# maxjiang216/corintho-ai

Hardware: AMD Instinct MI355X
Metric: self-play games/sec at 400 sims/move (higher is better)
Workload: dtype f32(f16x3)

## Files before the change

### corintho_ai_amd/csrc/engine.hip

```cpp
#include <math.h>
#include <stdio.h>
#include <stdlib.h>
#include <string.h>

#include <algorithm>
#include <memory>
#include <string>
#include <vector>

#include "analysis_host.h"
#include "game_logs.h"
#include "game_store.h"
#include "game_view.h"
#include "net_host.h"
#include "nn_group.h"
#include "pools.h"
#include "samples_host.h"

#ifdef CO_EMU
thread_local int co_emu_block_idx = 0;
#ifdef CO_SB_STATS
unsigned long long co_sb_stats[32];
unsigned long long co_sb_ply[8][8];
extern "C" unsigned long long *co_emu_sb_stats(void) { return co_sb_stats; }
extern "C" unsigned long long *co_emu_sb_ply(void) { return &co_sb_ply[0][0]; }
#endif
#endif

thread_local std::string g_last_error;
extern "C" const char *ca_last_error(void) { return g_last_error.c_str(); }
void co_set_last_error(const std::string &m) { g_last_error = m; }

struct ca_trainer {
  ca_config cfg;
  int G = 0, spe = 0;
  Stream stream;
  EngineParams P;
  GameStore store;
  GameView view;
  GameLogs logs;
  SampleExits samples;
  HostForward host_forward;
  AnalysisPositions positions;
  TourneyTables tour;
  int64_t iterations = 0;
  int32_t trainer_iteration = 0;
  bool scan_valid = false;
  int scan_valid_for = 0;
  int32_t last_total = 0;
  bool finished = false;
  bool any_error = false;
  bool net_used = false;
  std::unique_ptr<CoNet> nets[2];
  CallbackState callback{false, false, " in this generation; it cannot go on -- start a new one with ca_trainer_reset"};
  RunStats stats;
  FusedRun fused;
  bool host_cache = false;
  int host_cache_log2 = -1;
  int32_t host_rows = 0;
  HostNet host_net;
  HostPins pins;

  int dev() const { return cfg.device; }
  bool self_play_training() const { return !cfg.testing && !cfg.analyse && !tour.active(); }
  bool use_cache() const {
    if (cfg.eval_cache < 0 || tour.active() || cfg.analyse) return false;
    if (cfg.eval_cache > 0) return true;
    return nets[0] && nets[0]->flop_per_row() >= 1e6;
  }
  void invalidate() { scan_valid = view.valid = false; }
  size_t request_rows() const { return store.request_rows(spe); }
  const std::vector<GameCtl> &games() { return view.fetch(store, G, stream); }

  void init(const ca_config &c, TourneyTables tables = TourneyTables()) {
    cfg = c;
    tour = std::move(tables);
    if (cfg.analyse) {
      cfg.testing = 1;
      cfg.no_stagger = 1;
      cfg.game_base = cfg.total_games = 0;
    }
    if (cfg.max_searches <= 0) cfg.max_searches = 1600;
    if (cfg.searches_per_eval <= 0) cfg.searches_per_eval = 16;
    if (cfg.c_puct <= 0.0f) cfg.c_puct = 1.0f;
    G = cfg.num_games;
    spe = cfg.searches_per_eval;
    rt_set_device(cfg.device);
    stream.create();
    store.create(cfg, G, spe, self_play_training(), cfg.eval_cache >= 0 && !tour.active() && !cfg.analyse, stream);
    if (tour.active()) tour.create(store.R, stream);
    if (!cfg.analyse) reset_games(cfg.seed);
    rebind();
    fused.work_counter = store.work_counter.p;
    fused.nn_eval = store.nn_eval.p;
    fused.nn_probs = store.nn_probs.p;
    fused.stats = &stats;
    fused.stream = stream;
  }

  void rebind() {
    memset(&P, 0, sizeof P);
    store.bind(P, cfg, G, spe);
    logs.bind(P);
    tour.bind(P);
  }

  void reset_games(int32_t seed) {
    cfg.seed = seed;
    if (positions.given()) positions.write_terminal_rows(store.req.p, (size_t)spe * CO_STATE_STRIDE, stream);
    store.seed(cfg, G, tour.active() ? tour.match_seeds.data() : positions.given() ? positions.seed.data() : nullptr,
               [&](GameCtl &gc, int g) {
                 if (positions.given()) positions.place(gc, g);
               },
               stream);
    iterations = 0;
    trainer_iteration = 0;
    invalidate();
    last_total = 0;
    host_rows = 0;
    finished = false;
    const int64_t cache_clears = stats.cache_clears;
    stats = RunStats();
    stats.cache_clears = cache_clears;
    fused.cache_clean = false;
    callback.failed = false;
    for (auto &n : nets)
      if (n) n->clear_failure();
    logs.clear(stream);
  }

  void set_logging(const char *folder, int n) {
    if (tour.active() || cfg.analyse) throw CaError(CA_ERR_STATE, "per-game logs belong to Trainer games (self-play or arena)");
    if (iterations != 0 || trainer_iteration != 0) throw CaError(CA_ERR_STATE, "ca_trainer_set_logging: the games have started");
    if (n < 0) throw CaError(CA_ERR_ARG, "ca_trainer_set_logging: num_logged < 0");
    n -= cfg.game_base;
    if (n < 0) n = 0;
    if (n > G) n = G;
    if (n > store.R)
      throw CaError(CA_ERR_ARG, "ca_trainer_set_logging: " + std::to_string(n) + " logged games on " + std::to_string(store.R) +
                                        " resident slots -- a logged game must start in its own slot; raise ca_config.resident");
    std::vector<int> first(n);
    for (int g = 0; g < n; ++g) first[g] = g;
    set_log_records(first, GameLogs::game_paths(folder, cfg.game_base, n), false);
  }
  void set_log_records(const std::vector<int> &which, const std::vector<std::string> &paths, bool with_index) {
    logs.set_records(which, paths, with_index, G, stream);
    rebind();
  }
  void write_logs_once() {
    if (logs.pending()) logs.write(games(), stream);
  }

  EngineParams params(int to_play) const {
    EngineParams e = P;
    e.to_play = to_play;
    e.iteration = trainer_iteration;
    return e;
  }

  void scan(const EngineParams &e) { RT_LAUNCH(co_k_scan, 1, CO_WAVE, stream, e); }
  void compact(const EngineParams &e) { RT_LAUNCH(co_k_compact, store.R, CO_WAVE, stream, e); }
  void read_ctl(int to_play) {
    last_total = store.h_ctl[CO_CTL_ROWS];
    finished = store.h_ctl[CO_CTL_ALL_DONE] != 0;
    any_error = store.h_ctl[CO_CTL_ANY_ERROR] != 0;
    scan_valid_for = to_play;
    scan_valid = true;
  }
  void pack(int to_play) {
    if (scan_valid && scan_valid_for == to_play) return;
    const EngineParams e = params(to_play);
    scan(e);
    compact(e);
    rt_d2h(store.h_ctl, store.ctl.p, CO_CTL_WORDS * 4, stream);
    rt_sync(stream);
    read_ctl(to_play);
    if (finished && !any_error) write_logs_once();
  }
  bool poll_all_done(int to_play) {
    scan(params(to_play));
    int32_t d = 0;
    rt_d2h(&d, store.all_done.p, 4, stream);
    rt_sync(stream);
    return d != 0;
  }

  bool upload_answers(const float *evals, const float *probs, int32_t rows) {
    if (rows <= 0 || !evals || !probs) return false;
    rt_h2d(store.nn_eval.p, evals, (size_t)rows * 4, stream);
    rt_h2d(store.nn_probs.p, probs, (size_t)rows * CO_NUM_MOVES * 4, stream);
    return true;
  }

  void check_errors() {
    check_net_range();
    if (scan_valid && !any_error) return;
    throw_game_errors(games());
  }

  void step(const EngineParams &e) {
    launch_mcts_step(e, store.R, stream);
    ++stats.mcts_launches;
    invalidate();
    pack(e.to_play);
    check_errors();
  }
  void queue_iteration(const EngineParams &e, CoNet *net) {
    scan(e);
    if (net) {
      compact(e);
      net->forward(store.nn_in.p, store.R * spe, store.req_offset.p + store.R, store.nn_eval.p, store.nn_probs.p, stream);
      ++stats.nn_launches;
    }
    launch_mcts_step(e, store.R, stream);
    ++stats.mcts_launches;
    ++iterations;
  }
  void queue_grouped_iteration(CoNetGroup *group, GroupPlanner &planner, const int32_t *slot_model, int32_t *row_model) {
    const EngineParams e = params(CO_TO_PLAY_EVERY_MODEL);
    scan(e);
    compact(e);
    RT_LAUNCH(co_k_group_rows, store.R, CO_WAVE, stream, e, slot_model, row_model);
    planner.run(row_model, store.req_offset.p + store.R, stream);
    group->forward(store.nn_in.p, store.R * spe, planner.plan(), store.nn_eval.p, store.nn_probs.p, stream);
    ++stats.nn_launches;
    launch_mcts_step(e, store.R, stream);
    ++stats.mcts_launches;
    ++iterations;
  }
  void queued_iterations_done() {
    invalidate();
    check_errors();
  }
  void drain() {
    rt_sync(stream);
    invalidate();
  }

  void need_positions() const {
    if (cfg.analyse && !positions.given()) throw CaError(CA_ERR_STATE, "analysis trainer: ca_trainer_set_positions first");
  }
  bool do_iteration(const float *evals, const float *probs, int to_play) {
    need_positions();
    callback.need_none_failed("ca_trainer_do_iteration");
    if (host_cache) return host_cache_iteration(evals, probs, to_play);
    if (iterations > 0) {
      pack(to_play);
      if (last_total > 0 && !upload_answers(evals, probs, last_total))
        throw CaError(CA_ERR_ARG, "doIteration: null evaluations/probabilities");
    } else {
      rt_memset(store.req_offset.p, 0, ((size_t)store.R + 1) * 4, stream);
    }
    const EngineParams e = params(to_play);
    if (to_play == -1) ++trainer_iteration;
    ++iterations;
    step(e);
    return finished;
  }

  int32_t num_requests(int to_play) {
    if (host_cache) return host_cache_all_games(to_play), host_rows;
    pack(to_play);
    return last_total;
  }

  void write_requests(float *out, int to_play) {
    const int32_t n = num_requests(to_play);
    if (n == 0) return;
    rt_d2h(out, store.nn_in70.p, (size_t)n * CO_GAME_STATE_SIZE * 4, stream);
    rt_sync(stream);
  }

  void set_host_cache(int32_t log2_entries) {
    if ((log2_entries >= 1 && log2_entries <= 5) || log2_entries > 30)
      throw CaError(CA_ERR_ARG, "ca_trainer_set_host_cache: log2_entries must be negative (off), 0 (automatic) or 6..30, not " +
                                        std::to_string(log2_entries));
    const bool on = log2_entries >= 0;
    if (on && !self_play_training())
      throw CaError(CA_ERR_STATE, "ca_trainer_set_host_cache: the evaluation cache serves self-play training only, not a testing, "
                                  "analysis or tournament trainer");
    if (!on && !host_cache) return;
    if (iterations != 0)
      throw CaError(CA_ERR_STATE, "ca_trainer_set_host_cache: in the middle of a generation; switch before the first "
                                  "ca_trainer_do_iteration or after ca_trainer_reset");
    fused.release();
    host_cache = on;
    host_cache_log2 = log2_entries;
    fused.host_stepped = on;
    host_rows = 0;
    if (!on) return;
    if (!store.pend_key.p) {
      store.alloc_pend_keys(spe, stream);
      rebind();
      rt_sync(stream);
    }
    fused.spe = spe;
    fused.create(1, store.R, log2_entries);
    fused.cache_clean = false;
    host_net.rows_cap = request_rows();
    host_net.rows70 = store.nn_in70.p;
    host_net.ev_in = store.nn_eval.p;
    host_net.pr_in = store.nn_probs.p;
    host_net.d_ctl = store.ctl.p;
    host_net.h_ctl = &store.h_ctl[0];
    host_net.out_idx = nullptr;
  }
  void host_cache_all_games(int to_play) const {
    if (to_play != -1) throw CaError(CA_ERR_ARG, "host-driven protocol with the evaluation cache: to_play must be -1 (training)");
  }
  bool host_cache_iteration(const float *evals, const float *probs, int to_play) {
    host_cache_all_games(to_play);
    rt_stream_t st = fused.pools[0].st;
    if (host_rows > 0) {
      if (!evals || !probs) throw CaError(CA_ERR_ARG, "doIteration: null evaluations/probabilities");
      host_net.receive(evals, probs, host_rows, st);
      host_rows = 0;
    }
    EngineParams e = params(-1);
    e.step_budget = 0;
    e.step_budget_k16 = 0;
    host_net.scan_params = e;
    const int64_t n = fused.run(e, &host_net, 1, host_cache_log2, iterations > 0, 1);
    trainer_iteration += (int32_t)n;
    iterations += n;
    invalidate();
    stats.estimate_device_times(true);
    if (!fused.failure.empty()) throw CaError(CA_ERR_ENGINE, fused.failure);
    read_ctl(-1);
    const Pool::Seen &seen = fused.pools[0].seen[0];
    host_rows = (int32_t)std::min<size_t>(seen.evaluated, request_rows());
    stats.nn_rows += (int64_t)co_pack_rows(seen.pack);
    stats.nn_rows_evaluated += host_rows;
    check_errors();
    if (finished) write_logs_once();
    return finished;
  }

  int32_t need_samples(const char *what, int32_t cap_rows = INT32_MAX) {
    if (cfg.testing) throw CaError(CA_ERR_STATE, std::string(what) + " in testing mode");
    return samples.index(games(), cap_rows, stream);
  }
  void write_samples(float *gs, float *ev, float *pr) {
    const size_t n = (size_t)need_samples("writeSamples");
    if (n > 0) samples.write(P, G, n, gs, ev, pr, stream);
  }
  int32_t pack_samples_device(float *d_state_policy, float *d_outcome, int32_t cap_rows) {
    const int32_t n = need_samples("pack_samples", cap_rows);
    if (n > cap_rows) throw CaError(CA_ERR_ARG, "pack_samples: destination too small");
    if (n > 0) samples.pack(P, G, d_state_policy, d_outcome, stream);
    rt_sync(stream);
    return n;
  }
  void export_samples(float *state_policy, float *outcome) {
    const size_t n = (size_t)need_samples("export_samples");
    if (n > 0) samples.export_host(P, G, n, state_policy, outcome, stream);
  }

  void set_positions(const int32_t *boards, const int32_t *to_play, const int32_t *pieces, const int32_t *seeds) {
    if (!cfg.analyse) throw CaError(CA_ERR_STATE, "set_positions: not an analysis trainer (ca_config.analyse)");
    if (iterations > 0) throw CaError(CA_ERR_STATE, "set_positions after the first iteration");
    positions.set(boards, to_play, pieces, seeds, G, stream);
    reset_games(cfg.seed);
  }
  void analysis(int32_t *out) {
    if (!cfg.analyse) throw CaError(CA_ERR_STATE, "not an analysis trainer");
    AnalysisPositions::read(store.req.p, (size_t)spe * CO_STATE_STRIDE, games(), out, stream);
  }
  void finish_analysis() {
    if (!cfg.analyse) throw CaError(CA_ERR_STATE, "ca_trainer_finish: not an analysis trainer");
    if (iterations == 0) do_iteration(nullptr, nullptr, -1);
    EngineParams e = params(-1);
    e.force_choose = 1;
    step(e);
  }

  std::unique_ptr<CoNet> make_net(const NetSpec &spec, CallbackState *guard, const std::string &asker, const char *hint = "") {
    return spec.make(request_rows(), stream, guard, asker, hint);
  }
  void set_net(int slot, const NetSpec &spec, const char *who) {
    if (slot < 0 || slot > 1) throw CaError(CA_ERR_ARG, "net slot must be 0 or 1");
    install_net(slot, make_net(spec, &callback, ", this trainer", " (ca_trainer_request_rows)"), who);
  }

  void install_net(int slot, std::unique_ptr<CoNet> fresh, const char *who) {
    if (slot == 0 && !fused.pools.empty() && !host_cache) {
      std::unique_ptr<CoNet> old = std::move(nets[0]);
      nets[0] = std::move(fresh);
      const bool toggles = (fused.table.entries != 0) != use_cache();
      if (toggles && iterations > 0 && !finished) {
        nets[0] = std::move(old);
        throw CaError(CA_ERR_STATE, std::string(who) + ": this network turns the evaluation cache " +
                                            std::string(fused.table.entries ? "off" : "on") +
                                            " in the middle of a generation; finish or reset the generation first");
      }
      if (toggles) fused.release();
    } else {
      nets[slot] = std::move(fresh);
    }
    if (slot == 0) fused.cache_clean = false;
  }

  void check_callback() {
    for (int slot = 0; slot < 2; ++slot)
      if (nets[slot] && nets[slot]->callback_failed()) invalidate(), callback.check(nets[slot].get(), "slot " + std::to_string(slot));
  }

  void check_net_range() {
    if (!net_used) return;
    for (int slot = 0; slot < 2; ++slot) ::check_net_range(nets[slot].get(), stream, "network slot " + std::to_string(slot));
    net_used = false;
  }

  void net_forward_host(int slot, const float *states, int32_t n, float *evals, float *probs) {
    if (slot < 0 || slot > 1 || !nets[slot]) throw CaError(CA_ERR_STATE, "net slot not set");
    callback.need_none_failed("ca_trainer_net_forward");
    CoNet *net = nets[slot].get();
// ... 302 lines not shown
```

### corintho_ai_amd/csrc/game_store.h

```cpp
#pragma once
#include <string.h>

#include <algorithm>
#include <random>
#include <vector>

#include "host.h"
#include "kernels.h"
#include "pools.h"

struct GameStore {
  int R = 0;
  bool recycle = false;
  uint32_t cap_units = 0;
  DevBuf<GameCtl> games;
  DevBuf<TreeCtl> trees;
  DevBuf<uint4> arena, pend_key;
  DevBuf<int32_t> pend_src;
  DevBuf<uint32_t> pend_leaf, pend_path, pend_n, noise_raw, rng;
  DevBuf<int32_t> pend_depth, req_offset, trace, all_done;
  DevBuf<float> req, nn_in, nn_in70, nn_eval, nn_probs, samples;
  DevBuf<int32_t> row_idx;
  DevBuf<unsigned long long> row_counter, pack_counter, work_counter, prof, next_game;
  DevBuf<GameCtl> results;
  DevBuf<uint32_t> seeds_dev;
  DevBuf<int32_t> arena_state;
  DevBuf<int32_t> ctl;
  Pinned<int32_t> h_ctl;

  size_t request_rows(int spe) const { return (size_t)R * spe; }

  void alloc_pend_keys(int spe, rt_stream_t s) {
    pend_key.alloc(request_rows(spe), s);
    pend_src.alloc(request_rows(spe), s);
  }

  void create(const ca_config &cfg, int G, int spe, bool can_recycle, bool cache_words, rt_stream_t s) {
    uint32_t cap = cfg.arena_units;
    if (cap == 0) {
      uint64_t nodes = (uint64_t)cfg.max_searches * 14 + 64;
      cap = (uint32_t)std::min<uint64_t>(nodes * 40, 0x7FFFFFF0ull);
    }
    cap_units = cap;
    R = G;
    const size_t per_slot = (size_t)2 * ((size_t)cap + CO_ARENA_PAD) * sizeof(uint4) +
                            (size_t)spe * (CO_PATH_MAX * 4 + CO_NUM_MOVES * 4 + 2 * CO_STATE_STRIDE * 4 + CO_GAME_STATE_SIZE * 4 +
                                           CO_NUM_MOVES * 4 + 64) + CO_MT_N * 4 + 512;
    if (can_recycle && cfg.resident > 0 && cfg.resident < G) R = cfg.resident;
    if (can_recycle && cfg.resident == 0) {
      const size_t budget = rt_mem_free() / 8 * 5;
      const size_t per_game = (size_t)CO_MAX_PLIES * CO_SAMPLE_FLOATS * 4 + sizeof(GameCtl) + 8;
      if ((size_t)G * (per_slot + per_game) > budget) {
        size_t fit = budget > (size_t)G * per_game ? (budget - (size_t)G * per_game) / per_slot : 0;
        if (fit < 1) throw CaError(CA_ERR_DEVICE, "not enough device memory for a single resident game");
        R = (int)std::min<size_t>(fit, (size_t)G);
        if (R >= 512) R &= ~255;
      }
    }
    recycle = R < G;
    const size_t T = (size_t)2 * R, rows = request_rows(spe);
    games.alloc(R, s);
    trees.alloc(T, s);
    arena.alloc(T * ((size_t)cap + CO_ARENA_PAD), s);
    pend_leaf.alloc(rows, s);
    pend_depth.alloc(rows, s);
    pend_n.alloc(rows * 4, s);
    if (cache_words) alloc_pend_keys(spe, s);
    noise_raw.alloc(rows * CO_NUM_MOVES, s);
    pend_path.alloc(rows * CO_PATH_MAX, s);
    rng.alloc((size_t)R * CO_MT_N, s);
    req.alloc(rows * CO_STATE_STRIDE, s);
    req_offset.alloc((size_t)R + 1, s);
    nn_in.alloc(rows * CO_STATE_STRIDE, s);
    row_idx.alloc(rows, s);
    nn_in70.alloc(rows * CO_GAME_STATE_SIZE, s);
    ctl.alloc(CO_CTL_WORDS, s);
    h_ctl.alloc(CO_CTL_WORDS);
    nn_eval.alloc(rows, s);
    nn_probs.alloc(rows * CO_NUM_MOVES, s);
    if (!cfg.testing) samples.alloc((size_t)G * CO_MAX_PLIES * CO_SAMPLE_FLOATS, s);
    if (cfg.trace) trace.alloc((size_t)G * CO_TRACE_CAP, s);
    if (recycle) {
      results.alloc(G, s);
      seeds_dev.alloc(G, s);
    }
    next_game.alloc(1, s);
    all_done.alloc(1, s);
    row_counter.alloc(1, s);
    pack_counter.alloc((size_t)CO_PACK_STRIDE * CO_MAX_POOLS, s);
    work_counter.alloc((size_t)CO_WC_WORDS * CO_MAX_POOLS, s);
    arena_state.alloc(CO_AS_WORDS, s);
#ifdef CO_PROF
    prof.alloc((size_t)R * CO_NPROF + 24 + CO_NPROF, s);
#endif
  }

  template <class F>
  void seed(const ca_config &cfg, int G, const uint32_t *given, F &&place, rt_stream_t s) {
    size_t T = (size_t)2 * R;
    int total = cfg.total_games > 0 ? cfg.total_games : G;
    std::mt19937 gen((uint32_t)cfg.seed);
    std::vector<uint32_t> seeds(total);
    for (int i = 0; i < total; ++i) seeds[i] = (uint32_t)gen();
    std::vector<uint32_t> st((size_t)R * CO_MT_N);
    std::vector<GameCtl> hg(R);
    std::vector<TreeCtl> ht(T);
    for (int g = 0; g < R; ++g) {
      uint32_t *x = &st[(size_t)g * CO_MT_N];
      x[0] = given ? given[g] : seeds[cfg.game_base + g];
      for (int i = 1; i < CO_MT_N; ++i) x[i] = 1812433253u * (x[i - 1] ^ (x[i - 1] >> 30)) + (uint32_t)i;
      memset(&hg[g], 0, sizeof(GameCtl));
      hg[g].gid = g;
      hg[g].parity = (cfg.game_base + g) % 2;
      hg[g].rng_idx = CO_MT_N;
      hg[g].pos_meta = CO_META_START;
      place(hg[g], g);
    }
    for (size_t t = 0; t < T; ++t) {
      ht[t].root = CO_NONE;
      ht[t].searches_done = 0;
      ht[t].units_used = 0;
      ht[t].peak_units = 0;
    }
    rt_h2d(rng.p, st.data(), st.size() * 4, s);
    rt_h2d(games.p, hg.data(), hg.size() * sizeof(GameCtl), s);
    rt_h2d(trees.p, ht.data(), ht.size() * sizeof(TreeCtl), s);
    if (recycle) {
      rt_h2d(seeds_dev.p, seeds.data() + cfg.game_base, (size_t)G * 4, s);
      rt_memset(results.p, 0, (size_t)G * sizeof(GameCtl), s);
    }
    const unsigned long long first_unstarted = (unsigned long long)R;
    rt_h2d(next_game.p, &first_unstarted, 8, s);
    rt_memset(row_counter.p, 0, 8, s);
    rt_memset(pack_counter.p, 0, (size_t)8 * CO_PACK_STRIDE * CO_MAX_POOLS, s);
    rt_memset(work_counter.p, 0, (size_t)8 * CO_WC_WORDS * CO_MAX_POOLS, s);
    rt_memset(arena_state.p, 0, CO_AS_WORDS * 4, s);
    rt_sync(s);
  }

  void bind(EngineParams &P, const ca_config &cfg, int G, int spe) const {
    P.num_games = R;
    P.total_local = G;
    P.results = recycle ? results.p : nullptr;
    P.next_game = next_game.p;
    P.seeds = recycle ? seeds_dev.p : nullptr;
    P.max_searches = cfg.max_searches;
    P.searches_per_eval = spe;
    P.c_puct = cfg.c_puct;
    P.epsilon = cfg.epsilon;
    P.testing = cfg.testing;
    size_t div = (size_t)(cfg.total_games > 0 ? cfg.total_games : G) / (size_t)cfg.max_searches;
    if (div < 1) div = 1;
    P.stagger_div = (cfg.no_stagger || recycle) ? 0 : (int32_t)div;
    P.iteration = 0;
    P.to_play = -1;
    P.game_base = cfg.game_base;
    P.cap_units = cap_units;
    P.trace_on = cfg.trace;
    P.analyse = cfg.analyse;
    P.arena_state = nullptr;
    P.scan_phase = 0;
    P.games = games.p;
    P.trees = trees.p;
    P.arena = arena.p;
    P.pend_leaf = pend_leaf.p;
    P.pend_depth = pend_depth.p;
    P.pend_n = pend_n.p;
    P.pend_key = pend_key.p;
    P.pend_src = pend_src.p;
    P.noise_raw = noise_raw.p;
    P.pend_path = pend_path.p;
    P.rng = rng.p;
    P.req = req.p;
    P.req_offset = req_offset.p;
    P.nn_eval = nn_eval.p;
    P.nn_probs = nn_probs.p;
    P.nn_in = nn_in.p;
    P.row_idx = row_idx.p;
    P.nn_in70 = nn_in70.p;
    P.ctl = ctl.p;
    P.samples = samples.p;
    P.trace = trace.p;
    P.all_done = all_done.p;
    P.row_counter = nullptr;
    P.fused_pack = 0;
    P.defer_handover = 0;
    P.step_budget = cfg.step_budget > 0 ? cfg.step_budget : 0;
    P.step_budget_k16 = cfg.step_budget == 0 ? CO_STEP_BUDGET_K16 : cfg.step_budget < -1 ? -cfg.step_budget : 0;
    P.work_counter = nullptr;
    P.pool_lo = 0;
    P.pool_n = R;
    P.pool_row_base = 0;
    P.pack_counter = pack_counter.p;
    P.prof = prof.p;
  }

  int64_t peak_arena_units(rt_stream_t s) const {
    std::vector<TreeCtl> ht((size_t)2 * R);
    rt_d2h(ht.data(), trees.p, ht.size() * sizeof(TreeCtl), s);
    rt_sync(s);
    int64_t peak = 0;
    for (auto &x : ht) peak = std::max<int64_t>(peak, x.peak_units);
    return peak;
  }

  void read_prof(unsigned long long out[2 * CO_NPROF + 24], rt_stream_t s) const {
    if (!prof.p) throw CaError(CA_ERR_STATE, "not a -DCO_PROF build");
    for (int i = 0; i < 2 * CO_NPROF + 24; ++i) out[i] = 0;
    std::vector<unsigned long long> h((size_t)R * CO_NPROF);
    rt_d2h(h.data(), prof.p, h.size() * 8, s);
    rt_sync(s);
    for (int g = 0; g < R; ++g)
      for (int i = 0; i < CO_NPROF; ++i) out[i] += h[(size_t)g * CO_NPROF + i];
    rt_d2h(out + CO_NPROF, prof.p + (size_t)R * CO_NPROF, (size_t)(24 + CO_NPROF) * 8, s);
    rt_sync(s);
  }
};

struct TourneyTables {
  std::vector<PlayerCfg> host_pcfg;
  std::vector<uint32_t> match_seeds;
  bool exact_offsets = false;
  DevBuf<PlayerCfg> pcfg;
  DevBuf<int32_t> read_offset;

  bool active() const { return !host_pcfg.empty(); }
  void create(int R, rt_stream_t s) {
    pcfg.alloc(host_pcfg.size(), s);
    rt_h2d(pcfg.p, host_pcfg.data(), host_pcfg.size() * sizeof(PlayerCfg), s);
    read_offset.alloc((size_t)R, s);
  }
  void bind(EngineParams &P) const {
    P.pcfg = pcfg.p;
    P.read_offset = exact_offsets ? nullptr : read_offset.p;
  }
};
```

### corintho_ai_amd/csrc/kernels.h

```cpp
#pragma once
#include "mcts.h"

CO_CONST int32_t CO_SPACE_SYM[8][16] = CO_SPACE_SYM_INIT;
CO_CONST int32_t CO_MOVE_SYM[8][96] = CO_MOVE_SYM_INIT;

#ifdef CO_EMU
#define CO_K3_WAVES 1
#define CO_K3_WAVE_IN_BLOCK 0
#define CO_K3_BOUNDS
#else
#define CO_K3_BOUNDS __launch_bounds__(CO_K3_WPB * 64)
#define CO_K3_WAVES CO_K3_WPB
#define CO_K3_WAVE_IN_BLOCK (CO_K3_WPB > 1 ? __builtin_amdgcn_readfirstlane((int)(threadIdx.x >> 6)) : 0)
#endif
CO_K3_BOUNDS CO_KERNEL co_k_mcts_step(EngineParams P) {
  const int i = CO_BLOCK_IDX * CO_K3_WAVES + CO_K3_WAVE_IN_BLOCK;
  const int g = P.pool_lo + i;
  if (i < P.pool_n && g < P.num_games) co_mcts_step_wave(P, g);
}

CO_DEV int co_game_active(const EngineParams &P, int g, const GameCtl &gc, int tp) {
  if (gc.done) return 0;
  if (P.pcfg) return tp == CO_TO_PLAY_EVERY_MODEL || P.pcfg[2 * g + gc.to_play].model_id == tp;
  if (tp == 0 || tp == 1) return gc.to_play == (tp + gc.parity) % 2;
  return 1;
}

CO_KERNEL co_k_scan(EngineParams P) {
  int G = P.num_games;
  const int tp = P.arena_state ? P.arena_state[P.scan_phase == 0 ? CO_AS_NEXT : CO_AS_MODEL] : P.to_play;
  int chunk = (G + CO_WAVE - 1) / CO_WAVE;
  LV(int, csum);
  LV(int, nd);
  LV(int, er);
  FOR_LANES {
    int s = 0, notdone = 0, err = 0;
    for (int i = 0; i < chunk; ++i) {
      int g = lane * chunk + i;
      if (g < G) {
        GameCtl gc = P.games[g];
        if (co_game_active(P, g, gc, tp)) s += gc.n_pending;
        notdone += !gc.done;
        err |= gc.error;
      }
    }
    L(csum) = s;
    L(nd) = notdone;
    L(er) = err != 0;
  }
  int not_done = WAVE_SUM_I32(nd);
  int any_error = WAVE_BALLOT(er) != 0;
  WAVE_SHARED(int, cbase, CO_WAVE + 1);
  FOR_LANES { cbase[lane + 1] = L(csum); }
  WAVE_SYNC();
  int run = 0;
  LV(int, mybase);
  FOR_LANES { L(mybase) = 0; }
  for (int l = 0; l < CO_WAVE; ++l) {
    int v = cbase[l + 1];
    FOR_LANES {
      if (lane == l) L(mybase) = run;
    }
    run += v;
  }
  FOR_LANES {
    int s = L(mybase);
    for (int i = 0; i < chunk; ++i) {
      int g = lane * chunk + i;
      if (g < G) {
        GameCtl gc = P.games[g];
        P.req_offset[g] = s;
        if (co_game_active(P, g, gc, tp)) s += gc.n_pending;
      }
    }
    if (lane == 0 && P.read_offset) {
      int offset = 0;
      P.read_offset[0] = 0;
      for (int i = 1; i < G; ++i) {
        if (co_game_active(P, i, P.games[i], tp)) offset += P.games[i - 1].n_pending;
        P.read_offset[i] = offset;
      }
    }
    if (lane == 0) {
      P.req_offset[G] = run;
      P.all_done[0] = not_done == 0;
      if (P.ctl) {
        P.ctl[CO_CTL_ROWS] = run;
        P.ctl[CO_CTL_ALL_DONE] = not_done == 0;
        P.ctl[CO_CTL_ANY_ERROR] = any_error;
        P.ctl[CO_CTL_NOT_DONE] = not_done;
      }
      if (P.row_counter && (!P.arena_state || P.scan_phase == 1)) P.row_counter[0] += (unsigned long long)run;
      if (P.arena_state) {
        if (P.scan_phase == 0) {
          P.arena_state[CO_AS_MODEL] = tp;
        } else {
          P.arena_state[CO_AS_ROWS + (tp == 0 ? 1 : 0)] = run;
          P.arena_state[CO_AS_ROWS + (tp == 0 ? 0 : 1)] = 0;
          if (not_done != 0 && run == 0) {
            P.arena_state[CO_AS_NEXT] = 1 - tp;
            P.arena_state[CO_AS_EMPTY] += 1;
          } else {
            P.arena_state[CO_AS_NEXT] = tp;
            P.arena_state[CO_AS_EMPTY] = 0;
          }
        }
      }
    }
  }
}

CO_KERNEL co_k_compact(EngineParams P) {
  int g = CO_BLOCK_IDX;
  if (g >= P.num_games) return;
  GameCtl gc = P.games[g];
  if (!co_game_active(P, g, gc, P.arena_state ? P.arena_state[CO_AS_MODEL] : P.to_play)) return;
  int n = gc.n_pending;
  const float *src = P.req + (size_t)g * P.searches_per_eval * CO_STATE_STRIDE;
  float *dst = P.nn_in + (size_t)P.req_offset[g] * CO_STATE_STRIDE;
  int total = n * CO_STATE_STRIDE;
  FOR_LANES {
    for (int i = lane; i < total; i += CO_WAVE) dst[i] = src[i];
  }
  if (P.nn_in70) {
    float *d70 = P.nn_in70 + (size_t)P.req_offset[g] * CO_GAME_STATE_SIZE;
    int t70 = n * CO_GAME_STATE_SIZE;
    FOR_LANES {
      for (int i = lane; i < t70; i += CO_WAVE) d70[i] = src[(i / CO_GAME_STATE_SIZE) * CO_STATE_STRIDE + i % CO_GAME_STATE_SIZE];
    }
  }
}

CO_KERNEL co_k_expand_rows(const float *in70, float *out80, int rows, int nblocks) {
  FOR_LANES {
    int total = rows * CO_STATE_STRIDE;
    for (int i = CO_BLOCK_IDX * CO_WAVE + lane; i < total; i += CO_WAVE * nblocks) {
      int r = i / CO_STATE_STRIDE, c = i % CO_STATE_STRIDE;
      out80[i] = c < CO_GAME_STATE_SIZE ? in70[(size_t)r * CO_GAME_STATE_SIZE + c] : 0.0f;
    }
  }
}

#define CO_HOST_ROWS_FLOAT ((CO_BLOCK_IDX * CO_WAVES_PER_BLOCK + CO_WAVE_IN_BLOCK) * CO_WAVE + lane)
CO_KERNEL co_k_host_rows_out(const float *req, const int32_t *in_idx, const uint32_t *count, int cap_rows, float *out70) {
  const uint32_t have = count[0];
  const int rows = (int)(have < (uint32_t)cap_rows ? have : (uint32_t)cap_rows);
  const int total = cap_rows * CO_GAME_STATE_SIZE;
  FOR_LANES {
    const int e = CO_HOST_ROWS_FLOAT;
    if (e < total) {
      const int r = e / CO_GAME_STATE_SIZE, c = e - r * CO_GAME_STATE_SIZE;
      out70[e] = r < rows ? req[(size_t)(in_idx ? in_idx[r] : r) * CO_STATE_STRIDE + c] : 0.0f;
    }
  }
}
CO_KERNEL co_k_host_rows_in(const float *evals, const float *probs, const int32_t *out_idx, const uint32_t *count, int rows,
                            float *d_eval, float *d_probs, int eval_stride, int probs_stride) {
  const uint32_t have = count ? count[0] : (uint32_t)rows;
  const int total = (int)(have < (uint32_t)rows ? have : (uint32_t)rows) * (1 + CO_NUM_MOVES);
  FOR_LANES {
    const int e = CO_HOST_ROWS_FLOAT;
    if (e < total) {
      const int r = e / (1 + CO_NUM_MOVES), c = e - r * (1 + CO_NUM_MOVES);
      const size_t o = (size_t)(out_idx ? out_idx[r] : r);
      if (c == 0) d_eval[o * (size_t)eval_stride] = evals[r];
      else d_probs[o * (size_t)probs_stride + c - 1] = probs[(size_t)r * CO_NUM_MOVES + c - 1];
    }
  }
}

CO_KERNEL co_k_write_samples(EngineParams P, int n_games, const int32_t *sample_offset, const int32_t *meta, float *game_states,
                             float *eval_samples, float *prob_samples) {
  int g = CO_BLOCK_IDX;
  if (g >= n_games) return;
  const int n = meta[g] & 255, result = meta[g] >> 8;
  size_t off = (size_t)sample_offset[g];
  const float *smp = P.samples + (size_t)g * CO_MAX_PLIES * CO_SAMPLE_FLOATS;
  for (int i = n - 1; i >= 0; --i) {
    const float evaluation = co_sample_outcome(result, n, i);
    const float *st = smp + (size_t)i * CO_SAMPLE_FLOATS;
    const float *pol = st + CO_GAME_STATE_SIZE;
    for (int k = 0; k < CO_NUM_SYMMETRIES; ++k) {
      float *gs = game_states + ((off + i) * CO_NUM_SYMMETRIES + k) * CO_GAME_STATE_SIZE;
      float *ps = prob_samples + ((off + i) * CO_NUM_SYMMETRIES + k) * CO_NUM_MOVES;
      FOR_LANES {
        gs[lane] = st[CO_SPACE_SYM[k][lane / 4] * 4 + lane % 4];
        if (lane < CO_GAME_STATE_SIZE - 64) gs[64 + lane] = st[64 + lane];
        ps[lane] = pol[CO_MOVE_SYM[k][lane]];
        if (lane < CO_NUM_MOVES - 64) ps[64 + lane] = pol[CO_MOVE_SYM[k][64 + lane]];
        if (lane == 0) eval_samples[(off + i) * CO_NUM_SYMMETRIES + k] = evaluation;
      }
    }
  }
}

CO_KERNEL co_k_pack_samples(EngineParams P, int n_games, const int32_t *sample_offset, const int32_t *meta, float *state_policy,
                            float *outcome) {
  int g = CO_BLOCK_IDX;
  if (g >= n_games) return;
  const int n = meta[g] & 255, result = meta[g] >> 8;
  size_t off = (size_t)sample_offset[g];
  const float *smp = P.samples + (size_t)g * CO_MAX_PLIES * CO_SAMPLE_FLOATS;
  int total = n * CO_SAMPLE_FLOATS;
  FOR_LANES {
    for (int i = lane; i < total; i += CO_WAVE) state_policy[off * CO_SAMPLE_FLOATS + i] = smp[i];
    for (int i = lane; i < n; i += CO_WAVE) outcome[off + i] = co_sample_outcome(result, n, i);
  }
}

CO_KERNEL co_k_rules_batch(const uint64_t *boards, const uint32_t *metas, int n, uint32_t *masks, int32_t *lines) {
  int i = CO_BLOCK_IDX;
  if (i >= n) return;
  uint32_t lm[3];
  CoLanes K;
  co_lanes_init(K);
  int l = co_legal_moves(boards[i], metas[i], lm, K);
  FOR_LANES {
    if (lane < 3) masks[i * 3 + lane] = lm[lane];
    if (lane == 0) lines[i] = l;
  }
}

CO_KERNEL co_k_domove_batch(uint64_t *boards, uint32_t *metas, const int32_t *moves, int n, float *states) {
  int i = CO_BLOCK_IDX;
  if (i >= n) return;
  uint64_t b = boards[i];
  uint32_t m = metas[i];
  CoLanes K;
  co_lanes_init(K);
  if (moves[i] >= 0) co_do_move(&b, &m, moves[i], K);
  WAVE_SYNC();
  FOR_LANES {
    if (lane == 0) {
      boards[i] = b;
      metas[i] = m;
    }
  }
  co_write_state(b, m, states + (size_t)i * CO_STATE_STRIDE);
}

CO_KERNEL co_k_rules_rows(uint64_t *boards, uint32_t *metas, const int32_t *moves, int n, uint32_t *masks) {
  const int base = CO_BLOCK_IDX * 4;
  LV(uint32_t, blo);
  LV(uint32_t, bhi);
  LV(uint32_t, mt);
  LV(int, on);
  FOR_LANES {
    const int i = base + (lane >> 4);
    L(on) = i < n;
    uint64_t b = L(on) ? boards[i] : 0ull;
    uint32_t m = L(on) ? metas[i] : 0u;
    if (L(on) && moves[i] >= 0) co_do_move_lane(&b, &m, moves[i]);
    L(blo) = (uint32_t)b;
    L(bhi) = (uint32_t)(b >> 32);
    L(mt) = m;
  }
  LV(uint32_t, o0);
  LV(uint32_t, o1);
  LV(uint32_t, o2);
  WG_SHARED(uint32_t, lb, CO_LB_WORDS);
  co_line_breakers_to_lds(lb);
  LV(int, lines);
  co_legal_moves_rows(blo, bhi, mt, on, o0, o1, o2, lines, lb);
  FOR_LANES {
    const int i = base + (lane >> 4);
    if (L(on) && (lane & 15) == 0) {
      boards[i] = (uint64_t)L(blo) | ((uint64_t)L(bhi) << 32);
      metas[i] = L(mt);
      masks[i * 3 + 0] = L(o0);
      masks[i * 3 + 1] = L(o1);
      masks[i * 3 + 2] = L(o2);
    }
  }
}

CO_KERNEL co_k_rng_draw(uint32_t *mt, int32_t *idx_io, int n, int chunk, uint32_t *out) {
  int idx = idx_io[0];
  int done = 0;
  while (done < n) {
    int cnt = n - done < chunk ? n - done : chunk;
    LV(uint32_t, r);
    CO_MT_DRAW(mt, idx, cnt, r);
    FOR_LANES {
      if (lane < cnt) out[done + lane] = L(r);
    }
    done += cnt;
  }
  FOR_LANES {
    if (lane == 0) idx_io[0] = idx;
  }
}

CO_KERNEL co_k_fp_probe(const float *in, int n, float *out) {
  FOR_LANES {
    int i = CO_BLOCK_IDX * CO_WAVE + lane;
    if (i < n) {
      const float *x = in + (size_t)i * 8;
      float c_puct = x[0], visits = x[1], eval = x[2], p9 = x[3], denom = x[4], cv = x[5], sum = x[6], eps = x[7];
      float v_sqrt = (float)((double)c_puct * co_sqrt_f64((double)visits));
      float prob = p9 * denom;
      float pv = prob * v_sqrt;
      int icv = (int)cv;
      double a, b;
      if ((float)icv == cv && icv >= 1 && icv < 32768) {
        a = co_div_small(-(double)eval, cv);
        b = co_div_small((double)pv, cv + 1.0f);
      } else {
        a = -1.0 * (double)eval / (double)cv;
        b = (double)pv / ((double)cv + 1.0);
      }
      float one_minus = (float)1 - eps;
      float *o = out + (size_t)i * 8;
      o[0] = v_sqrt;
      o[1] = (float)(a + b);
      o[2] = pv;
      o[3] = (float)(1.0 / (double)sum * (double)one_minus);
      o[4] = (float)(1.0 / (double)sum * (double)eps);
      o[5] = 511.0f / sum;
      o[6] = (float)(1.0 / (double)(float)(int)cv);
      float xq = p9 * (511.0f / sum);
      float fl = __builtin_truncf(xq);
      int q = (int)fl;
      if (xq - fl >= 0.5f) q += 1;
      o[7] = (float)q;
    }
  }
}
```

### corintho_ai_amd/csrc/probes.h

```cpp
#pragma once
#include <memory>
#include <vector>

#include "net_host.h"

struct ca_net {
  int device = 0;
  Stream stream;
  std::unique_ptr<CoNet> net;
  DevBuf<float> rows80;
  Event used;
  rt_stream_t used_on = {};
  bool used_once = false;
  int dev() const { return device; }

  void forward_device(const float *d_states, int32_t rows_cap, const int32_t *d_rows, float *d_evals, float *d_probs, void *stream_arg) {
    if (!d_states || !d_rows || !d_evals || !d_probs) throw CaError(CA_ERR_ARG, "ca_net_forward_device: null buffer");
    if (rows_cap < 0 || (size_t)rows_cap > net->max_rows()) throw CaError(CA_ERR_ARG, "ca_net_forward_device: more rows than the net's max_rows");
    if (rows_cap == 0) return;
    launch(d_states, rows_cap, rows_cap, d_rows, d_evals, d_probs, CoNetIO(), stream_arg, "ca_net_forward_device");
  }

  void forward_device_io(const float *d_states, int32_t state_rows, int32_t rows_cap, const int32_t *d_rows, float *d_evals,
                         float *d_probs, const CoNetIO &io, void *stream_arg) {
    const char *who = "ca_net_forward_device_io";
    if (!d_states || !d_rows || !d_evals || !d_probs) throw CaError(CA_ERR_ARG, std::string(who) + ": null buffer");
    if (rows_cap < 0 || (size_t)rows_cap > net->max_rows() || state_rows < 0 || (size_t)state_rows > net->max_rows())
      throw CaError(CA_ERR_ARG, std::string(who) + ": more rows than the net's max_rows");
    if (!io.in_idx && state_rows < rows_cap)
      throw CaError(CA_ERR_ARG, std::string(who) + ": without in_idx the launch reads rows_cap rows, state_rows is fewer");
    if (io.eval_stride < 1 || io.probs_stride < CO_NET_NUM_MOVES)
      throw CaError(CA_ERR_ARG, std::string(who) + ": eval_stride < 1 or probs_stride < 96");
    if (rows_cap == 0) return;
    launch(d_states, state_rows, rows_cap, d_rows, d_evals, d_probs, io, stream_arg, who);
  }

  void launch(const float *d_states, int32_t state_rows, int32_t rows_cap, const int32_t *d_rows, float *d_evals, float *d_probs,
              const CoNetIO &io, void *stream_arg, const char *who) {
    const rt_stream_t s = stream_arg ? (rt_stream_t)(intptr_t)stream_arg : (rt_stream_t)stream;
    if (used_once && used_on != s) rt_stream_wait(s, used);
    expand_rows(d_states, rows80.p, state_rows, s);
    net->forward(rows80.p, rows_cap, d_rows, d_evals, d_probs, s, io);
    rt_event_record(used, s);
    used_on = s;
    used_once = true;
    if (!stream_arg) {
      rt_sync(s);
      check_net_range(net.get(), s, who);
    }
  }
};

extern "C" int ca_net_create(int device, int kind, const float *weights, size_t n_floats, int32_t max_rows, ca_net **out) {
  return on_device_stream(device, [&](Stream &s) {
    if (!out || !weights || max_rows <= 0) throw CaError(CA_ERR_ARG, "ca_net_create: null argument or max_rows < 1");
    *out = nullptr;
    auto n = std::make_unique<ca_net>();
    n->device = device;
    n->stream = std::move(s);
    n->used.create();
    n->net = NetSpec(kind, weights, n_floats).make((size_t)max_rows, n->stream, nullptr);
    n->rows80.alloc((size_t)max_rows * CO_STATE_STRIDE, n->stream);
    rt_sync(n->stream);
    *out = n.release();
  });
}
extern "C" int ca_net_forward_device(ca_net *n, const float *d_states, int32_t rows_cap, const int32_t *d_rows, float *d_evals,
                                     float *d_probs, void *stream) {
  return co_guard(n, [&] { n->forward_device(d_states, rows_cap, d_rows, d_evals, d_probs, stream); });
}
extern "C" int ca_net_forward_device_io(ca_net *n, const float *d_states, int32_t state_rows, int32_t rows_cap, const int32_t *d_rows,
                                        const int32_t *d_in_idx, const int32_t *d_out_idx, float *d_evals, int32_t eval_stride,
                                        float *d_probs, int32_t probs_stride, int32_t alone, void *stream) {
  return co_guard(n, [&] {
    CoNetIO io;
    io.in_idx = d_in_idx, io.out_idx = d_out_idx, io.eval_stride = eval_stride, io.probs_stride = probs_stride, io.alone = alone != 0;
    n->forward_device_io(d_states, state_rows, rows_cap, d_rows, d_evals, d_probs, io, stream);
  });
}
extern "C" void ca_net_destroy(ca_net *n) { delete n; }


extern "C" int ca_rules_legal_moves(int device, const uint64_t *boards, const uint32_t *metas, int32_t n, uint32_t *masks,
                                    int32_t *is_lines) {
  return on_device_stream(device, [&](Stream &ts) {
    DevBuf<uint64_t> b;
    DevBuf<uint32_t> m, mk;
    DevBuf<int32_t> ln;
    b.upload(boards, n, ts); m.upload(metas, n, ts); mk.alloc((size_t)n * 3, ts); ln.alloc(n, ts);
    RT_LAUNCH(co_k_rules_batch, n, CO_WAVE, ts, (const uint64_t *)b.p, (const uint32_t *)m.p, n, mk.p, ln.p);
    rt_d2h(masks, mk.p, (size_t)n * 12, ts);
    rt_d2h(is_lines, ln.p, (size_t)n * 4, ts);
    rt_sync(ts);
  });
}

extern "C" int ca_rules_do_move(int device, uint64_t *boards, uint32_t *metas, const int32_t *moves, int32_t n, float *states) {
  return on_device_stream(device, [&](Stream &ts) {
    DevBuf<uint64_t> b;
    DevBuf<uint32_t> m;
    DevBuf<int32_t> mv;
    DevBuf<float> st;
    b.upload(boards, n, ts); m.upload(metas, n, ts); mv.upload(moves, n, ts); st.alloc((size_t)n * CO_STATE_STRIDE, ts);
    RT_LAUNCH(co_k_domove_batch, n, CO_WAVE, ts, b.p, m.p, (const int32_t *)mv.p, n, st.p);
    std::vector<float> tmp((size_t)n * CO_STATE_STRIDE);
    rt_d2h(boards, b.p, (size_t)n * 8, ts);
    rt_d2h(metas, m.p, (size_t)n * 4, ts);
    rt_d2h(tmp.data(), st.p, tmp.size() * 4, ts);
    rt_sync(ts);
    for (int i = 0; i < n; ++i)
      memcpy(states + (size_t)i * CO_GAME_STATE_SIZE, &tmp[(size_t)i * CO_STATE_STRIDE], CO_GAME_STATE_SIZE * 4);
  });
}

extern "C" int ca_rules_rows(int device, uint64_t *boards, uint32_t *metas, const int32_t *moves, int32_t n, uint32_t *masks) {
  return on_device_stream(device, [&](Stream &ts) {
    DevBuf<uint64_t> b;
    DevBuf<uint32_t> m, mk;
    DevBuf<int32_t> mv;
    b.upload(boards, n, ts); m.upload(metas, n, ts); mv.upload(moves, n, ts); mk.alloc((size_t)n * 3, ts);
    RT_LAUNCH(co_k_rules_rows, (n + 3) / 4, CO_WAVE, ts, b.p, m.p, (const int32_t *)mv.p, n, mk.p);
    rt_d2h(boards, b.p, (size_t)n * 8, ts);
    rt_d2h(metas, m.p, (size_t)n * 4, ts);
    rt_d2h(masks, mk.p, (size_t)n * 12, ts);
    rt_sync(ts);
  });
}

extern "C" int ca_rng_draw(int device, uint32_t seed, int32_t n, int32_t chunk, uint32_t *out) {
  return on_device_stream(device, [&](Stream &ts) {
    if (chunk < 1 || chunk > CO_WAVE) throw CaError(CA_ERR_ARG, "chunk must be 1..64");
    std::vector<uint32_t> x(CO_MT_N);
    x[0] = seed;
    for (int i = 1; i < CO_MT_N; ++i) x[i] = 1812433253u * (x[i - 1] ^ (x[i - 1] >> 30)) + (uint32_t)i;
    DevBuf<uint32_t> mt, o;
    DevBuf<int32_t> idx;
    const int32_t i0 = CO_MT_N;
    mt.upload(x.data(), CO_MT_N, ts); idx.upload(&i0, 1, ts); o.alloc(n, ts);
    RT_LAUNCH(co_k_rng_draw, 1, CO_WAVE, ts, mt.p, idx.p, n, chunk, o.p);
    rt_d2h(out, o.p, (size_t)n * 4, ts);
    rt_sync(ts);
  });
}

extern "C" int ca_fp_probe(int device, const float *in, int32_t n, float *out) {
  return on_device_stream(device, [&](Stream &ts) {
    DevBuf<float> di, dout;
    di.upload(in, (size_t)n * 8, ts); dout.alloc((size_t)n * 8, ts);
    RT_LAUNCH(co_k_fp_probe, (n + CO_WAVE - 1) / CO_WAVE, CO_WAVE, ts, (const float *)di.p, n, dout.p);
    rt_d2h(out, dout.p, (size_t)n * 32, ts);
    rt_sync(ts);
  });
}
```

### corintho_ai_amd/csrc/rng.h

```cpp
#pragma once
#include "engine_defs.h"
#include "wave.h"

CO_DEV uint32_t co_mt_temper(uint32_t y) {
  y ^= y >> 11;
  y ^= (y << 7) & 0x9d2c5680u;
  y ^= (y << 15) & 0xefc60000u;
  y ^= y >> 18;
  return y;
}

CO_DEV void co_mt_seed(uint32_t *mt, uint32_t seed) {
  FOR_LANES {
    if (lane == 0) {
      uint32_t x = seed;
      mt[0] = x;
      for (int i = 1; i < CO_MT_N; ++i) {
        x = 1812433253u * (x ^ (x >> 30)) + (uint32_t)i;
        mt[i] = x;
      }
    }
  }
  WAVE_SYNC();
}

CO_DEV void co_mt_twist(uint32_t *mt) {
  for (int c = 0; c < (CO_MT_N + CO_WAVE - 1) / CO_WAVE; ++c) {
    LV(uint32_t, nv);
    FOR_LANES {
      int i = c * CO_WAVE + lane;
      if (i < CO_MT_N) {
        int i1 = i + 1 == CO_MT_N ? 0 : i + 1;
        int im = i + 397 >= CO_MT_N ? i + 397 - CO_MT_N : i + 397;
        uint32_t y = (mt[i] & 0x80000000u) | (mt[i1] & 0x7fffffffu);
        L(nv) = mt[im] ^ (y >> 1) ^ ((y & 1u) ? 0x9908b0dfu : 0u);
      }
    }
    WAVE_SYNC();
    FOR_LANES {
      int i = c * CO_WAVE + lane;
      if (i < CO_MT_N) mt[i] = L(nv);
    }
    WAVE_SYNC();
  }
}

#define CO_MT_STAGE 640
CO_DEV void co_mt_stage_load(const uint32_t *mt, uint32_t *st) {
  LV(uint32_t, x[10]);
  FOR_LANES {
#pragma unroll
    for (int c = 0; c < 10; ++c) {
      const int i = c * CO_WAVE + lane;
      L(x[c]) = mt[i < CO_MT_N ? i : 0];
    }
  }
  FOR_LANES {
#pragma unroll
    for (int c = 0; c < 10; ++c) {
      const int i = c * CO_WAVE + lane;
      if (i < CO_MT_N) st[i] = L(x[c]);
    }
  }
  WAVE_SYNC();
}
CO_DEV void co_mt_twist_staged(uint32_t *mt, uint32_t *st) {
  for (int c = 0; c < (CO_MT_N + CO_WAVE - 1) / CO_WAVE; ++c) {
    LV(uint32_t, nv);
    FOR_LANES {
      int i = c * CO_WAVE + lane;
      if (i < CO_MT_N) {
        int i1 = i + 1 == CO_MT_N ? 0 : i + 1;
        int im = i + 397 >= CO_MT_N ? i + 397 - CO_MT_N : i + 397;
        uint32_t y = (st[i] & 0x80000000u) | (st[i1] & 0x7fffffffu);
        L(nv) = st[im] ^ (y >> 1) ^ ((y & 1u) ? 0x9908b0dfu : 0u);
      }
    }
    WAVE_SYNC();
    FOR_LANES {
      int i = c * CO_WAVE + lane;
      if (i < CO_MT_N) st[i] = L(nv);
    }
    WAVE_SYNC();
  }
  LV(uint32_t, x[10]);
  FOR_LANES {
#pragma unroll
    for (int c = 0; c < 10; ++c) {
      const int i = c * CO_WAVE + lane;
      L(x[c]) = st[i < CO_MT_N ? i : 0];
    }
  }
  FOR_LANES {
#pragma unroll
    for (int c = 0; c < 10; ++c) {
      const int i = c * CO_WAVE + lane;
      if (i < CO_MT_N) mt[i] = L(x[c]);
    }
  }
}

#define CO_MT_DRAW(mt, idx, n, outvar)                          \
  do {                                                          \
    int _done = 0;                                              \
    while (_done < (n)) {                                       \
      if ((idx) >= CO_MT_N) {                                   \
        co_mt_twist(mt);                                        \
        (idx) = 0;                                              \
      }                                                         \
      int _take = (n)-_done;                                    \
      if (_take > CO_MT_N - (idx)) _take = CO_MT_N - (idx);     \
      FOR_LANES {                                               \
        int _j = lane - _done;                                  \
        if (_j >= 0 && _j < _take) L(outvar) = co_mt_temper((mt)[(idx) + _j]); \
      }                                                         \
      (idx) += _take;                                           \
      _done += _take;                                           \
    }                                                           \
  } while (0)

CO_DEV uint32_t co_mt_next(uint32_t *mt, int *idx) {
  if (*idx >= CO_MT_N) {
    co_mt_twist(mt);
    *idx = 0;
  }
  uint32_t y = co_mt_temper(mt[*idx]);
  *idx += 1;
  return y;
}
```

Measured before the change: 10710.

## Move game and RNG seeding from host to a device kernel

```diff
diff --git a/corintho_ai_amd/csrc/engine.hip b/corintho_ai_amd/csrc/engine.hip
--- a/corintho_ai_amd/csrc/engine.hip
+++ b/corintho_ai_amd/csrc/engine.hip
@@ -109,9 +109,7 @@
     cfg.seed = seed;
     if (positions.given()) positions.write_terminal_rows(store.req.p, (size_t)spe * CO_STATE_STRIDE, stream);
     store.seed(cfg, G, tour.active() ? tour.match_seeds.data() : positions.given() ? positions.seed.data() : nullptr,
-               [&](GameCtl &gc, int g) {
-                 if (positions.given()) positions.place(gc, g);
-               },
+               positions.given(), [&](GameCtl &gc, int g) { positions.place(gc, g); },
                stream);
     iterations = 0;
     trainer_iteration = 0;
diff --git a/corintho_ai_amd/csrc/game_store.h b/corintho_ai_amd/csrc/game_store.h
--- a/corintho_ai_amd/csrc/game_store.h
+++ b/corintho_ai_amd/csrc/game_store.h
@@ -24,6 +24,9 @@
   DevBuf<unsigned long long> row_counter, pack_counter, work_counter, prof, next_game;
   DevBuf<GameCtl> results;
   DevBuf<uint32_t> seeds_dev;
+  Pinned<uint32_t> h_seeds;
+  Event seeds_sent;
+  bool seeded = false;
   DevBuf<int32_t> arena_state;
   DevBuf<int32_t> ctl;
   Pinned<int32_t> h_ctl;
@@ -93,49 +96,51 @@
 #ifdef CO_PROF
     prof.alloc((size_t)R * CO_NPROF + 24 + CO_NPROF, s);
 #endif
+    h_seeds.alloc(G);
+    seeds_sent.create();
   }
 
   template <class F>
-  void seed(const ca_config &cfg, int G, const uint32_t *given, F &&place, rt_stream_t s) {
-    size_t T = (size_t)2 * R;
-    int total = cfg.total_games > 0 ? cfg.total_games : G;
-    std::mt19937 gen((uint32_t)cfg.seed);
-    std::vector<uint32_t> seeds(total);
-    for (int i = 0; i < total; ++i) seeds[i] = (uint32_t)gen();
-    std::vector<uint32_t> st((size_t)R * CO_MT_N);
-    std::vector<GameCtl> hg(R);
-    std::vector<TreeCtl> ht(T);
-    for (int g = 0; g < R; ++g) {
-      uint32_t *x = &st[(size_t)g * CO_MT_N];
-      x[0] = given ? given[g] : seeds[cfg.game_base + g];
-      for (int i = 1; i < CO_MT_N; ++i) x[i] = 1812433253u * (x[i - 1] ^ (x[i - 1] >> 30)) + (uint32_t)i;
-      memset(&hg[g], 0, sizeof(GameCtl));
-      hg[g].gid = g;
-      hg[g].parity = (cfg.game_base + g) % 2;
-      hg[g].rng_idx = CO_MT_N;
-      hg[g].pos_meta = CO_META_START;
-      place(hg[g], g);
-    }
-    for (size_t t = 0; t < T; ++t) {
-      ht[t].root = CO_NONE;
-      ht[t].searches_done = 0;
-      ht[t].units_used = 0;
-      ht[t].peak_units = 0;
-    }
-    rt_h2d(rng.p, st.data(), st.size() * 4, s);
-    rt_h2d(games.p, hg.data(), hg.size() * sizeof(GameCtl), s);
-    rt_h2d(trees.p, ht.data(), ht.size() * sizeof(TreeCtl), s);
-    if (recycle) {
-      rt_h2d(seeds_dev.p, seeds.data() + cfg.game_base, (size_t)G * 4, s);
-      rt_memset(results.p, 0, (size_t)G * sizeof(GameCtl), s);
-    }
-    const unsigned long long first_unstarted = (unsigned long long)R;
-    rt_h2d(next_game.p, &first_unstarted, 8, s);
-    rt_memset(row_counter.p, 0, 8, s);
-    rt_memset(pack_counter.p, 0, (size_t)8 * CO_PACK_STRIDE * CO_MAX_POOLS, s);
-    rt_memset(work_counter.p, 0, (size_t)8 * CO_WC_WORDS * CO_MAX_POOLS, s);
-    rt_memset(arena_state.p, 0, CO_AS_WORDS * 4, s);
-    rt_sync(s);
+  void seed(const ca_config &cfg, int G, const uint32_t *given, bool placed, F &&place, rt_stream_t s) {
+    if (seeded) rt_event_sync(seeds_sent);
+    if (given) {
+      for (int g = 0; g < G; ++g) h_seeds[g] = given[g];
+    } else {
+      const int total = cfg.total_games > 0 ? cfg.total_games : G;
+      std::mt19937 gen((uint32_t)cfg.seed);
+      for (int i = 0; i < total; ++i) {
+        const uint32_t x = (uint32_t)gen();
+        if (i >= cfg.game_base && i < cfg.game_base + G) h_seeds[i - cfg.game_base] = x;
+      }
+    }
+    uint32_t *d_seeds = recycle ? seeds_dev.p : pend_leaf.p;
+    rt_h2d(d_seeds, &h_seeds[0], (size_t)G * 4, s);
+    rt_event_record(seeds_sent, s);
+    seeded = true;
+    SeedCounters C;
+    C.next_game = next_game.p;
+    C.row_counter = row_counter.p;
+    C.pack_counter = pack_counter.p;
+    C.work_counter = work_counter.p;
+    C.arena_state = arena_state.p;
+    C.pack_words = CO_PACK_STRIDE * CO_MAX_POOLS;
+    C.work_words = CO_WC_WORDS * CO_MAX_POOLS;
+    const int per_block = CO_WAVE * CO_WAVES_PER_BLOCK;
+    RT_LAUNCH(co_k_seed_games, (R + per_block - 1) / per_block, per_block, s, games.p, trees.p, rng.p, (const uint32_t *)d_seeds, R, (int)cfg.game_base, C);
+    if (recycle) rt_memset(results.p, 0, (size_t)G * sizeof(GameCtl), s);
+    if (placed) {
+      std::vector<GameCtl> hg(R);
+      for (int g = 0; g < R; ++g) {
+        memset(&hg[g], 0, sizeof(GameCtl));
+        hg[g].gid = g;
+        hg[g].parity = (cfg.game_base + g) % 2;
+        hg[g].rng_idx = CO_MT_N;
+        hg[g].pos_meta = CO_META_START;
+        place(hg[g], g);
+      }
+      rt_h2d(games.p, hg.data(), hg.size() * sizeof(GameCtl), s);
+      rt_sync(s);
+    }
   }
 
   void bind(EngineParams &P, const ca_config &cfg, int G, int spe) const {
diff --git a/corintho_ai_amd/csrc/kernels.h b/corintho_ai_amd/csrc/kernels.h
--- a/corintho_ai_amd/csrc/kernels.h
+++ b/corintho_ai_amd/csrc/kernels.h
@@ -165,6 +165,40 @@
       const size_t o = (size_t)(out_idx ? out_idx[r] : r);
       if (c == 0) d_eval[o * (size_t)eval_stride] = evals[r];
       else d_probs[o * (size_t)probs_stride + c - 1] = probs[(size_t)r * CO_NUM_MOVES + c - 1];
+    }
+  }
+}
+
+struct SeedCounters {
+  unsigned long long *next_game, *row_counter, *pack_counter, *work_counter;
+  int32_t *arena_state;
+  int pack_words, work_words;
+};
+CO_KERNEL co_k_seed_games(GameCtl *games, TreeCtl *trees, uint32_t *rng, const uint32_t *seeds, int R, int game_base, SeedCounters C) {
+  FOR_LANES {
+    const int g = CO_HOST_ROWS_FLOAT;
+    if (g < R) {
+      GameCtl gc = {};
+      gc.gid = g;
+      gc.parity = (game_base + g) % 2;
+      gc.rng_idx = CO_MT_N;
+      gc.pos_meta = CO_META_START;
+      games[g] = gc;
+      TreeCtl tc;
+      tc.root = CO_NONE;
+      tc.searches_done = 0;
+      tc.units_used = 0;
+      tc.peak_units = 0;
+      trees[2 * (size_t)g] = tc;
+      trees[2 * (size_t)g + 1] = tc;
+      co_mt_seed_lane(rng + (size_t)g * CO_MT_N, seeds[g]);
+    }
+    if (g == 0) {
+      C.next_game[0] = (unsigned long long)R;
+      C.row_counter[0] = 0ull;
+      for (int i = 0; i < C.pack_words; ++i) C.pack_counter[i] = 0ull;
+      for (int i = 0; i < C.work_words; ++i) C.work_counter[i] = 0ull;
+      for (int i = 0; i < CO_AS_WORDS; ++i) C.arena_state[i] = 0;
     }
   }
 }
diff --git a/corintho_ai_amd/csrc/probes.h b/corintho_ai_amd/csrc/probes.h
--- a/corintho_ai_amd/csrc/probes.h
+++ b/corintho_ai_amd/csrc/probes.h
@@ -130,14 +130,16 @@
 extern "C" int ca_rng_draw(int device, uint32_t seed, int32_t n, int32_t chunk, uint32_t *out) {
   return on_device_stream(device, [&](Stream &ts) {
     if (chunk < 1 || chunk > CO_WAVE) throw CaError(CA_ERR_ARG, "chunk must be 1..64");
-    std::vector<uint32_t> x(CO_MT_N);
-    x[0] = seed;
-    for (int i = 1; i < CO_MT_N; ++i) x[i] = 1812433253u * (x[i - 1] ^ (x[i - 1] >> 30)) + (uint32_t)i;
-    DevBuf<uint32_t> mt, o;
-    DevBuf<int32_t> idx;
-    const int32_t i0 = CO_MT_N;
-    mt.upload(x.data(), CO_MT_N, ts); idx.upload(&i0, 1, ts); o.alloc(n, ts);
-    RT_LAUNCH(co_k_rng_draw, 1, CO_WAVE, ts, mt.p, idx.p, n, chunk, o.p);
+    DevBuf<uint32_t> mt, o, sd;
+    DevBuf<GameCtl> gc;
+    DevBuf<TreeCtl> tc;
+    DevBuf<unsigned long long> cnt;
+    DevBuf<int32_t> as;
+    sd.upload(&seed, 1, ts); mt.alloc(CO_MT_N, ts); gc.alloc(1, ts); tc.alloc(2, ts); cnt.alloc(4, ts); as.alloc(CO_AS_WORDS, ts);
+    o.alloc(n, ts);
+    SeedCounters sc = {cnt.p, cnt.p + 1, cnt.p + 2, cnt.p + 3, as.p, 1, 1};
+    RT_LAUNCH(co_k_seed_games, 1, CO_WAVE * CO_WAVES_PER_BLOCK, ts, gc.p, tc.p, mt.p, (const uint32_t *)sd.p, 1, 0, sc);
+    RT_LAUNCH(co_k_rng_draw, 1, CO_WAVE, ts, mt.p, &gc.p->rng_idx, n, chunk, o.p);
     rt_d2h(out, o.p, (size_t)n * 4, ts);
     rt_sync(ts);
   });
diff --git a/corintho_ai_amd/csrc/rng.h b/corintho_ai_amd/csrc/rng.h
--- a/corintho_ai_amd/csrc/rng.h
+++ b/corintho_ai_amd/csrc/rng.h
@@ -10,16 +10,17 @@
   return y;
 }
 
+CO_DEV void co_mt_seed_lane(uint32_t *mt, uint32_t seed) {
+  uint32_t x = seed;
+  mt[0] = x;
+  for (int i = 1; i < CO_MT_N; ++i) {
+    x = 1812433253u * (x ^ (x >> 30)) + (uint32_t)i;
+    mt[i] = x;
+  }
+}
 CO_DEV void co_mt_seed(uint32_t *mt, uint32_t seed) {
   FOR_LANES {
-    if (lane == 0) {
-      uint32_t x = seed;
-      mt[0] = x;
-      for (int i = 1; i < CO_MT_N; ++i) {
-        x = 1812433253u * (x ^ (x >> 30)) + (uint32_t)i;
-        mt[i] = x;
-      }
-    }
+    if (lane == 0) co_mt_seed_lane(mt, seed);
   }
   WAVE_SYNC();
 }
```

Result: no change. 10810 (median of 6 runs) (+0.9%).
